# manips-sai-org/sai-primitives

Measured on AMD Instinct MI355X. Metric: control-cycles/sec (whole node), 7-DoF 2-task hierarchy, batch=4096, higher is better.
Workload: dtype f64

## Files before the change

### sai-primitives_amd/csrc/saip_kernel_oct.hip

```cpp
#include <hip/hip_runtime.h>
#include <math.h>

#include "saip_device.h"
#include "saip_dynamics_oct_body.h"
#include "saip_fk.h"
#include "saip_law.h"
#include "saip_oct_common.h"
#define SAIP_WG_SYNC()                                          \
	do {                                                        \
		__builtin_amdgcn_fence(__ATOMIC_RELEASE, "wavefront");  \
		__builtin_amdgcn_wave_barrier();                        \
		__builtin_amdgcn_fence(__ATOMIC_ACQUIRE, "wavefront");  \
	} while (0)
#include "saip_wg_cycle.h"

namespace saip {

#if defined(SAIP_STAMP_OCT)
__device__ unsigned long long saip_stamps_oct[1024 * 64];
#define STAMP(i)                                                                              \
	do {                                                                                      \
		__builtin_amdgcn_sched_barrier(0);                                                    \
		if (blockIdx.x < 1024 && (threadIdx.x & 63) == 0) saip_stamps_oct[blockIdx.x * 64 + (threadIdx.x >> 6) * 32 + (i)] = __builtin_amdgcn_s_memtime(); \
		__builtin_amdgcn_sched_barrier(0);                                                    \
	} while (0)
#else
#define STAMP(i)
#endif

struct OctInst {
	union {
		double X[8][12];
		struct {
			double T1[6][8], A[8][8], Am[8][8], Lam[8][8];
			double N1[8][8];
		};
	};
	double M[8][8];
	double zo[8][6];
	double J[6][8];
	double vec[13][8];
	double ist[10];
};
static_assert(sizeof(OctInst) % 256 == 16, "instance stride must be 2 (mod 32) doubles");
static_assert(sizeof(OctInst) * 8 * 4 <= 160 * 1024, "four wavefronts per CU (one LDS block each, also with two wavefronts per instance group)");

template <int R>
__device__ __forceinline__ void oct_jacobi_n(double (&A)[R][R], double (&V)[R][R], const int lane) {
	static_assert(R == 4 || R == 6, "even sizes with at most three pairs per round");
	constexpr int NP = R / 2, RM = R - 1;
	const int r = octl_r(lane), m = r & 1;
	auto rotation = [](const double apq, const double app, const double aqq, double& cs, double& sn, double& tn) {
		const double d = aqq - app, b2 = 2.0 * apq;
		const double x = fma(d, d, b2 * b2);
		const bool rot = x > 1e-300;
		const double h = rot ? x * oct_rsqrt(x) : 1.0;
		const double tm = fabs(b2) * oct_rcp(fabs(d) + h);
		tn = rot ? (((d >= 0.0) == (b2 >= 0.0)) ? tm : -tm) : 0.0;
		cs = oct_rsqrt(fma(tn, tn, 1.0));
		sn = tn * cs;
	};
	double vrow[R];
	UNR for (int j = 0; j < R; j++) vrow[j] = (j == r) ? 1.0 : 0.0;
	for (int sweep = 0; sweep < 12; sweep++) {
		double off = 0.0, dg = 0.0;
		UNR for (int p = 0; p < R; p++) {
			dg = fma(A[p][p], A[p][p], dg);
			UNR for (int q = p + 1; q < R; q++) off = fma(A[p][q], A[p][q], off);
		}
		if (!__any(off > 1e-32 * dg)) break;
		UNR for (int t = 0; t < RM; t++) {
			double apq = 0.0, app = 0.0, aqq = 0.0;
			UNR for (int j = 0; j < NP; j++) {
				const int a_ = j == 0 ? t : (t + j) % RM, b_ = j == 0 ? RM : (t + RM - j) % RM;
				const int p = a_ < b_ ? a_ : b_, q = a_ < b_ ? b_ : a_;
				const bool mine = m == j;
				apq = mine ? A[p][q] : apq;
				app = mine ? A[p][p] : app;
				aqq = mine ? A[q][q] : aqq;
			}
			double cs, sn, tn, cs2 = 1.0, sn2 = 0.0, tn2 = 0.0;
			rotation(apq, app, aqq, cs, sn, tn);
			if (NP == 3) {
				const int a_ = (t + 2) % RM, b_ = (t + RM - 2) % RM;
				const int p = a_ < b_ ? a_ : b_, q = a_ < b_ ? b_ : a_;
				rotation(A[p][q], A[p][p], A[q][q], cs2, sn2, tn2);
			}
			UNR for (int j = 0; j < NP; j++) {
				const int a_ = j == 0 ? t : (t + j) % RM, b_ = j == 0 ? RM : (t + RM - j) % RM;
				const int p = a_ < b_ ? a_ : b_, q = a_ < b_ ? b_ : a_;
				double c, s_, tj;
				if (j == 0) { c = oct_dpp<0x44>(cs); s_ = oct_dpp<0x44>(sn); tj = oct_dpp<0x44>(tn); }
				else if (j == 1) { c = oct_dpp<0xEE>(cs); s_ = oct_dpp<0xEE>(sn); tj = oct_dpp<0xEE>(tn); }
				else { c = cs2; s_ = sn2; tj = tn2; }
				const double apq_j = A[p][q];
				UNR for (int k = 0; k < R; k++) {
					if (k != p && k != q) {
						const double akp = A[k][p], akq = A[k][q];
						const double np_ = c * akp - s_ * akq, nq_ = s_ * akp + c * akq;
						A[k][p] = np_;
						A[p][k] = np_;
						A[k][q] = nq_;
						A[q][k] = nq_;
					}
				}
				A[p][p] = fma(-tj, apq_j, A[p][p]);
				A[q][q] = fma(tj, apq_j, A[q][q]);
				A[p][q] = 0.0;
				A[q][p] = 0.0;
				const double vp = vrow[p], vq = vrow[q];
				vrow[p] = c * vp - s_ * vq;
				vrow[q] = s_ * vp + c * vq;
			}
		}
	}
	UNR for (int i = 0; i < R; i++)
		UNR for (int c = 0; c < R; c++) V[i][c] = __shfl(vrow[c], octl_src(lane, i));
}
__device__ __forceinline__ void oct_jacobi4(double (&A)[4][4], double (&V)[4][4], const int lane) { oct_jacobi_n<4>(A, V, lane); }
__device__ __forceinline__ void oct_spd_inverse4(const double (&A)[4][4], double (&Ainv)[4][4]) { oct_spd_inverse_n<4>(A, Ainv); }


__device__ __forceinline__ void oct_fk_frame(const ModelDev& md, const int rr, const int r, const double q, double (&Tw)[12]) {
	const double* R0 = md.R0[rr];
	const double ax = md.axis[rr][0], ay = md.axis[rr][1], az = md.axis[rr][2];
	if (md.jtype[rr] == 1) {
		double s, c;
		sincos_joint(q, &s, &c);
		const double v = 1.0 - c;
		const double Rq[9] = {c + ax * ax * v,      ax * ay * v - az * s, ax * az * v + ay * s,
							  ay * ax * v + az * s, c + ay * ay * v,      ay * az * v - ax * s,
							  az * ax * v - ay * s, az * ay * v + ax * s, c + az * az * v};
		UNR for (int i = 0; i < 3; i++)
			UNR for (int j = 0; j < 3; j++) Tw[3 * i + j] = R0[3 * i] * Rq[j] + R0[3 * i + 1] * Rq[3 + j] + R0[3 * i + 2] * Rq[6 + j];
		UNR for (int e = 0; e < 3; e++) Tw[9 + e] = md.p0[rr][e];
	} else {
		UNR for (int e = 0; e < 9; e++) Tw[e] = R0[e];
		const double a[3] = {ax, ay, az};
		double d[3];
		oct_mat3_vec(R0, a, d);
		UNR for (int e = 0; e < 3; e++) Tw[9 + e] = md.p0[rr][e] + d[e] * q;
	}
	OCT_FRAME_STEP(1, Tw)
	OCT_FRAME_STEP(2, Tw)
	OCT_FRAME_STEP(4, Tw)
}


template <bool DUO>
__device__ __forceinline__ void oct_sync() {
	if (DUO) {
		__builtin_amdgcn_fence(__ATOMIC_RELEASE, "wavefront");
		__builtin_amdgcn_wave_barrier();
		__builtin_amdgcn_fence(__ATOMIC_ACQUIRE, "wavefront");
	} else {
		__syncthreads();
	}
}

template <bool FULL, int GJ, int ROLE, int NN = 7>
__device__ __forceinline__ bool oct_cycle_body(const CycleParams& P, OctInst* smem, OctInst* smemA, OctInst* smemB, int* wgflags = nullptr, double* lawc = nullptr) {
	constexpr bool DUO = ROLE != 0;
	constexpr bool roleA = ROLE != 2, roleB = ROLE != 1;
	constexpr int N = NN;
	constexpr bool CF = !FULL && GJ == 0;
	constexpr bool BROWS = DUO && CF;
	auto flag_wait = [&](const int k) {
		int it = 0, v = 0;
		while ((v = __hip_atomic_load(wgflags + k, __ATOMIC_RELAXED, __HIP_MEMORY_SCOPE_WORKGROUP)) == 0 && ++it < 200000) __builtin_amdgcn_s_sleep(1);
		__builtin_amdgcn_fence(__ATOMIC_ACQUIRE, "workgroup");
		return v;
	};
	auto flag_set = [&](const int k, const int v) {
		__builtin_amdgcn_fence(__ATOMIC_RELEASE, "workgroup");
		if ((threadIdx.x & 63) == 0) __hip_atomic_store(wgflags + k, v, __ATOMIC_RELAXED, __HIP_MEMORY_SCOPE_WORKGROUP);
	};
	bool lost = false;
	static_assert(NN == 7 || (FULL && GJ == 2), "6- and 8-dof chains: the general instantiation only");
	const int lane = threadIdx.x & 63;
	const int r = octl_r(lane), grp = octl_grp(lane);
	const int rr = r < N ? r : N - 1;
	const bool act = r < N;
	OctInst& sm = smem[grp];
	OctInst& smA = smemA[grp];
	OctInst& smB = smemB[grp];
	const int b_raw = (int)blockIdx.x * 8 + grp;
	const bool live = b_raw < P.B;
	const int b = live ? b_raw : P.B - 1;
	const size_t ld = P.ld;
	const ModelDev& md = *P.model;
	const TaskDev& mf = P.tasks[0];
	const TaskDev& jt = P.tasks[1];
	const int kmf = FULL ? mf.k : 6;
	const int mf_dec_v = mf.decoupling, jt_dec_v = jt.decoupling;
	const bool trunc_mode = FULL && GJ == 2 && P.oct_truncate;

	STAMP(0);
	const double q_r = P.q[(size_t)rr * ld + b];
	const double dq_r = P.dq[(size_t)rr * ld + b];
	const int jtype_r = md.jtype[rr];
	double R0v[9], p0v[3], axv[3];
	UNR for (int e = 0; e < 9; e++) R0v[e] = md.R0[rr][e];
	UNR for (int e = 0; e < 3; e++) {
		p0v[e] = md.p0[rr][e];
		axv[e] = md.axis[rr][e];
	}
	double comv[3] = {0, 0, 0}, inev[6] = {0, 0, 0, 0, 0, 0}, mass_r = 0.0;
	if (ROLE == 0) {
		UNR for (int e = 0; e < 3; e++) comv[e] = md.com[rr][e];
		UNR for (int e = 0; e < 6; e++) inev[e] = md.inertia[rr][e];
		mass_r = md.mass[rr];
	}
	double gl0 = 0.0, gl1 = 0.0, gl2 = 0.0;
	if (roleB) {
		gl0 = saip_ldg(P.goal2[0], (size_t)r * ld + b);
		gl1 = saip_ldg(P.goal2[0], (size_t)(8 + r) * ld + b);
		gl2 = saip_ldg(P.goal2[0], (size_t)(16 + r) * ld + b);
	}
	const double gl3 = (roleB && FULL && mf.general_law && r < 6) ? saip_ldg(P.goal2[0], (size_t)(24 + r) * ld + b) : 0.0;
	static_assert(offsetof(TaskDev, Ppos) == offsetof(TaskDev, Bm) + 36 * 8 && offsetof(TaskDev, Pori) == offsetof(TaskDev, Bm) + 45 * 8 &&
					  offsetof(TaskDev, sig_p) == offsetof(TaskDev, Bm) + 54 * 8 && offsetof(TaskDev, sig_o) == offsetof(TaskDev, Bm) + 63 * 8 &&
					  offsetof(TaskDev, kp_pos) == offsetof(TaskDev, Bm) + 72 * 8 && offsetof(TaskDev, ki_ori) == offsetof(TaskDev, Bm) + 87 * 8,
				  "the law constants are one contiguous run");
	double lc0 = 0.0, lc1 = 0.0;
	if (FULL && roleB) {
		const double* lsrc = reinterpret_cast<const double*>(reinterpret_cast<const char*>(&mf) + offsetof(TaskDev, Bm));
		lc0 = lsrc[lane];
		lc1 = lsrc[lane < 26 ? 64 + lane : 89];
	}
	const int mj = GJ == 1 ? jt.m : N;
	const int rj = GJ == 1 ? (r < mj ? r : 0) : rr;
	double jg_q = 0.0, jg_dq = 0.0, jg_ddq = 0.0;
	if (roleA) {
		jg_q = saip_ldg(P.goal2[1], (size_t)rj * ld + b);
		jg_dq = saip_ldg(P.goal2[1], (size_t)(mj + rj) * ld + b);
		jg_ddq = saip_ldg(P.goal2[1], (size_t)(2 * mj + rj) * ld + b);
	}

#define OCT_REQUEST_STATE(SFX)                                                                                          \
	const bool track_mf##SFX = (mf.has_ki || P.integ_always), track_jt##SFX = (jt.has_ki || P.integ_always);            \
	double mfi_pre##SFX = 0.0, jti_pre##SFX = 0.0;                                                                      \
	if (roleB && track_mf##SFX && r < 6) mfi_pre##SFX = saip_ldg(P.integ2[0], (size_t)r * ld + b);                                   \
	if (roleA && track_jt##SFX) jti_pre##SFX = saip_ldg(P.integ2[1], (size_t)(GJ == 1 ? rj : rr) * ld + b);                          \
	double jkp_r##SFX = 0.0, jkv_r##SFX = 0.0, jki_r##SFX = 0.0;  \
	if (roleA && GJ != 1) {                                                                                             \
		jkp_r##SFX = jt.kp[rr];                                                                                         \
		jkv_r##SFX = jt.kv[rr];                                                                                         \
		jki_r##SFX = jt.ki[rr];                                                                                         \
	}
	double jt_ie_new = 0.0;
	OCT_REQUEST_STATE(_e)

	STAMP(1);
	double Tw[12];
	{
		const double* R0 = R0v;
		const double ax = axv[0], ay = axv[1], az = axv[2];
		if (jtype_r == 1) {
			double s, c;
			sincos_joint(q_r, &s, &c);
			if (md.all_axis_z) {
				UNR for (int i = 0; i < 3; i++) {
					Tw[3 * i] = R0[3 * i] * c + R0[3 * i + 1] * s;
					Tw[3 * i + 1] = R0[3 * i + 1] * c - R0[3 * i] * s;
					Tw[3 * i + 2] = R0[3 * i + 2];
				}
			} else {
				const double v = 1.0 - c;
				const double Rq[9] = {c + ax * ax * v,      ax * ay * v - az * s, ax * az * v + ay * s,
									  ay * ax * v + az * s, c + ay * ay * v,      ay * az * v - ax * s,
									  az * ax * v - ay * s, az * ay * v + ax * s, c + az * az * v};
				UNR for (int i = 0; i < 3; i++)
					UNR for (int j = 0; j < 3; j++) Tw[3 * i + j] = R0[3 * i] * Rq[j] + R0[3 * i + 1] * Rq[3 + j] + R0[3 * i + 2] * Rq[6 + j];
			}
			UNR for (int e = 0; e < 3; e++) Tw[9 + e] = p0v[e];
		} else {
			UNR for (int e = 0; e < 9; e++) Tw[e] = R0[e];
			const double a[3] = {ax, ay, az};
			double d[3];
// ... 100 lines not shown
		const double c0 = z[1] * rz - z[2] * ry, c1 = z[2] * rx - z[0] * rz, c2 = z[0] * ry - z[1] * rx;
		const double jw[6] = {on ? (rev ? c0 : z[0]) : 0.0, on ? (rev ? c1 : z[1]) : 0.0, on ? (rev ? c2 : z[2]) : 0.0,
							  (on && rev) ? z[0] : 0.0,    (on && rev) ? z[1] : 0.0,    (on && rev) ? z[2] : 0.0};
		UNR for (int a = 0; a < 6; a++) jwc[a] = act ? jw[a] : 0.0;
		if (FULL && !mf.bm_identity) {
			UNR for (int a = 0; a < 6; a++) {
				double sj = 0.0;
				UNR for (int e = 0; e < 6; e++) sj = fma(lawc[e * 6 + a], jw[e], sj);
				sm.J[a][r] = sj;
			}
		} else {
			UNR for (int a = 0; a < 6; a++) sm.J[a][r] = jw[a];
		}
	}
	double fi_pre = 0.0;
	if (roleA && GJ != 1) {
		const double e = q_r - jg_q;
		double ie = track_jt ? jti_pre : 0.0;
		ie += e * jt.dt;
		jt_ie_new = ie;
		if (jt.vel_sat) {
			double vdes = -jkp_r * jt.kvinv[rr] * e - jki_r * jt.kvinv[rr] * ie;
			vdes = fmin(fmax(vdes, -jt.sat[rr]), jt.sat[rr]);
			fi_pre = -jkv_r * (dq_r - vdes);
		} else {
			fi_pre = -jkp_r * e - jkv_r * (dq_r - jg_dq) - jki_r * ie;
		}
	}
	if (BROWS) oct_sync<DUO>();
	else if (DUO && !trunc_mode) __syncthreads();
	else oct_sync<DUO>();
	STAMP(3);
	double mi[N] = {}, mb[N] = {};
	int eclamp = 0;
	double cclamp = 0.0;
	bool general_bie = false;
	if (roleA) {
		double L[N][N], dinv[N];
		UNR for (int i = 0; i < N; i++)
			UNR for (int j = 0; j <= i; j++) L[i][j] = sm.M[i][j];
		if (P.any_bie) {
			int nclamp = 0;
			UNR for (int e = 0; e < N; e++) {
				const double ce = P.bie_thr - L[e][e];
				if (ce > 0.0) {
					nclamp++;
					eclamp = e;
					cclamp = ce;
				}
			}
			general_bie = __any(nclamp > 1);
		}
		if (general_bie) {
			double Lb[N][N], dinvb[N];
			UNR for (int i = 0; i < N; i++)
				UNR for (int j = 0; j <= i; j++) Lb[i][j] = (i == j) ? fmax(L[i][j], P.bie_thr) : L[i][j];
			oct_cholesky<N>(L, dinv);
			oct_cholesky<N>(Lb, dinvb);
			oct_solve_unit<N>(L, dinv, rr, mi);
			oct_solve_unit<N>(Lb, dinvb, rr, mb);
		} else {
			oct_cholesky<N>(L, dinv);
			oct_solve_unit<N>(L, dinv, rr, mi);
			UNR for (int j = 0; j < N; j++) mb[j] = mi[j];
		}
	}
	const bool rank1_bie = P.any_bie && !general_bie;
	auto park_minv = [&]() {
		if (ROLE == 1) {
			UNR for (int j = 0; j < N; j++) sm.N1[r][j] = mi[j];
		}
		if (roleA && rank1_bie && r == eclamp) {
			UNR for (int j = 0; j < N; j++) sm.vec[3][j] = mi[j];
		}
	};
	if (!CF) park_minv();
	STAMP(4);
	double Jf[6][N];
	unsigned keep_bits_b = 0x3fu;
	if (DUO && trunc_mode && ROLE == 1) {
		__syncthreads();
		keep_bits_b = (unsigned)smB.vec[6][7];
	}
	if (!(BROWS && ROLE == 1)) {
		UNR for (int a = 0; a < 6; a++)
			UNR for (int j = 0; j < N; j++) Jf[a][j] = (ROLE == 1 ? smB : sm).J[a][j];
	}
	double vw[6] = {0, 0, 0, 0, 0, 0};
	if (roleB) {
		double dqa[N];
		UNR for (int j = 0; j < N; j++) dqa[j] = sm.vec[0][j];
		UNR for (int a = 0; a < 6; a++) {
			double s = 0.0;
			UNR for (int j = 0; j < N; j++) s = fma(Jf[a][j], dqa[j], s);
			vw[a] = s;
		}
		if (FULL && !mf.bm_identity) {
			UNR for (int a = 0; a < 6; a++) vw[a] = octl_sum(jwc[a] * dq_r);
		}
	}
	STAMP(5);
	double Fum6[6], Ff6[6] = {0, 0, 0, 0, 0, 0};
	STAMP(6);
	bool singular = false, truncated = false, blended_i = false;
	const bool strategies_on = GJ == 0 && mf.sing_handling && mf.sing_strategies && mf.sh != nullptr;
	double G[6][6], U6[6][6];
	bool keepm[6] = {true, true, true, true, true, true};
	double LG[6][6], dG[6];
	double zcf[N] = {}, wcf[N] = {}, zzcf = 0.0;
	auto form_z = [&](const double (&Lg)[6][6], const double (&dg)[6]) {
		double jc6[6], x6[6], xb[6], prr = 1.0;
		UNR for (int a = 0; a < 6; a++) jc6[a] = (ROLE == 1 ? smB : sm).J[a][rr];
		oct_solve<6>(Lg, dg, jc6, x6);
		UNR for (int a = 0; a < 6; a++) prr = fma(-jc6[a], x6[a], prr);
		double bestw = act ? prr : -1.0;
		int jbw = r;
#define OCT_ARGMAX_STEP(CTRL)                                                                                   \
	{                                                                                                           \
		const double ob = oct_dpp<CTRL>(bestw);                                                                 \
		const int oj = __builtin_amdgcn_update_dpp(0, jbw, CTRL, 0xF, 0xF, true);                               \
		const bool take = ob > bestw || (ob == bestw && oj < jbw);                                              \
		bestw = take ? ob : bestw;                                                                              \
		jbw = take ? oj : jbw;                                                                                  \
	}
		OCT_ARGMAX_STEP(OCT_BFLY0)
		OCT_ARGMAX_STEP(OCT_BFLY1)
		OCT_ARGMAX_STEP(OCT_BFLY2)
#undef OCT_ARGMAX_STEP
		const int src = octl_src(lane, jbw);
		UNR for (int a = 0; a < 6; a++) xb[a] = __shfl(x6[a], src);
		double z_own = (rr == jbw) ? 1.0 : 0.0;
		UNR for (int a = 0; a < 6; a++) z_own = fma(-jc6[a], xb[a], z_own);
		UNR for (int j = 0; j < N; j++) {
			zcf[j] = __shfl(z_own, octl_src(lane, j));
			zzcf = fma(zcf[j], zcf[j], zzcf);
		}
	};
	auto run_law = [&]() {
		double ip[3] = {0, 0, 0}, io[3] = {0, 0, 0}, Fum[6], G24[24];
		UNR for (int e = 0; e < 24; e++) G24[e] = sm.vec[10 + (e >> 3)][e & 7];
		if (track_mf) {
			UNR for (int i = 0; i < 3; i++) {
				ip[i] = sm.ist[i];
				io[i] = sm.ist[3 + i];
			}
		}
		if (FULL && mf.general_law) {
			double G30[30], Ff[6] = {0, 0, 0, 0, 0, 0};
			UNR for (int e = 0; e < 24; e++) G30[e] = G24[e];
			UNR for (int e = 0; e < 6; e++) G30[24 + e] = sm.vec[5][e];
			law_motion_force_general<false>(&mf, vw, pw, Rc, G30, ip, io, (double*)nullptr, Fum, Ff);
			UNR for (int a = 0; a < 6; a++) Ff6[a] = Ff[a];
		} else if (FULL && !mf.bm_identity) {
			double v[3], w[3], e3[3], tmp[3], Fw[6];
			UNR for (int i = 0; i < 3; i++) {
				v[i] = lawc[36 + 3 * i] * vw[0] + lawc[36 + 3 * i + 1] * vw[1] + lawc[36 + 3 * i + 2] * vw[2];
				w[i] = lawc[45 + 3 * i] * vw[3] + lawc[45 + 3 * i + 1] * vw[4] + lawc[45 + 3 * i + 2] * vw[5];
			}
			UNR for (int i = 0; i < 3; i++) e3[i] = pw[i] - G24[i];
			UNR for (int i = 0; i < 3; i++) ip[i] += (lawc[54 + 3 * i] * e3[0] + lawc[54 + 3 * i + 1] * e3[1] + lawc[54 + 3 * i + 2] * e3[2]) * mf.dt;
			UNR for (int i = 0; i < 3; i++) tmp[i] = G24[18 + i] - lawc[72 + i] * e3[i] - lawc[75 + i] * (v[i] - G24[12 + i]) - lawc[78 + i] * ip[i];
			UNR for (int i = 0; i < 3; i++) Fw[i] = lawc[54 + 3 * i] * tmp[0] + lawc[54 + 3 * i + 1] * tmp[1] + lawc[54 + 3 * i + 2] * tmp[2];
			double oe[3] = {0, 0, 0};
			UNR for (int c = 0; c < 3; c++) {
				const double a0 = Rc[c], a1 = Rc[3 + c], a2 = Rc[6 + c], b0 = G24[3 + c], b1 = G24[6 + c], b2 = G24[9 + c];
				oe[0] -= 0.5 * (a1 * b2 - a2 * b1);
				oe[1] -= 0.5 * (a2 * b0 - a0 * b2);
				oe[2] -= 0.5 * (a0 * b1 - a1 * b0);
			}
			double dphi[3];
			UNR for (int i = 0; i < 3; i++) dphi[i] = lawc[63 + 3 * i] * oe[0] + lawc[63 + 3 * i + 1] * oe[1] + lawc[63 + 3 * i + 2] * oe[2];
			UNR for (int i = 0; i < 3; i++) io[i] += dphi[i] * mf.dt;
			UNR for (int i = 0; i < 3; i++) tmp[i] = G24[21 + i] - lawc[81 + i] * dphi[i] - lawc[84 + i] * (w[i] - G24[15 + i]) - lawc[87 + i] * io[i];
			UNR for (int i = 0; i < 3; i++) Fw[3 + i] = lawc[63 + 3 * i] * tmp[0] + lawc[63 + 3 * i + 1] * tmp[1] + lawc[63 + 3 * i + 2] * tmp[2];
			UNR for (int a = 0; a < 6; a++) {
				double sf = 0.0;
				UNR for (int e = 0; e < 6; e++) sf = fma(lawc[0 + e * 6 + a], Fw[e], sf);
				Fum[a] = sf;
			}
		} else {
		double e3[3];
		UNR for (int i = 0; i < 3; i++) e3[i] = pw[i] - G24[i];
		UNR for (int i = 0; i < 3; i++) ip[i] = fma(e3[i], mf.dt, ip[i]);
		UNR for (int i = 0; i < 3; i++) Fum[i] = G24[18 + i] - mf.kp_pos[i] * e3[i] - mf.kv_pos[i] * (vw[i] - G24[12 + i]) - mf.ki_pos[i] * ip[i];
		double oe[3] = {0, 0, 0};
		UNR for (int c = 0; c < 3; c++) {
			const double a0 = Rc[c], a1 = Rc[3 + c], a2 = Rc[6 + c], b0 = G24[3 + c], b1 = G24[6 + c], b2 = G24[9 + c];
			oe[0] -= 0.5 * (a1 * b2 - a2 * b1);
			oe[1] -= 0.5 * (a2 * b0 - a0 * b2);
			oe[2] -= 0.5 * (a0 * b1 - a1 * b0);
		}
		UNR for (int i = 0; i < 3; i++) io[i] = fma(oe[i], mf.dt, io[i]);
		UNR for (int i = 0; i < 3; i++) Fum[3 + i] = G24[21 + i] - mf.kp_ori[i] * oe[i] - mf.kv_ori[i] * (vw[3 + i] - G24[15 + i]) - mf.ki_ori[i] * io[i];
		}
		if (track_mf && r == 0) {
			UNR for (int i = 0; i < 3; i++) {
				sm.ist[i] = ip[i];
				sm.ist[3 + i] = io[i];
			}
		}
		if (trunc_mode) {
			double fh[6];
			UNR for (int a = 0; a < 6; a++) {
				double sf = 0.0;
				UNR for (int i = 0; i < 6; i++) sf = fma(U6[i][a], Fum[i], sf);
				fh[a] = keepm[a] ? sf : 0.0;
			}
			UNR for (int a = 0; a < 6; a++) Fum[a] = fh[a];
		}
		UNR for (int a = 0; a < 6; a++) Fum6[a] = Fum[a];
	};
	if (roleB && CF) run_law();
	if (roleB) {
		double tr = 0.0;
		UNR for (int a = 0; a < 6; a++)
			UNR for (int c = 0; c <= a; c++) {
				double s = 0.0;
				UNR for (int j = 0; j < N; j++) s = fma(Jf[a][j], Jf[c][j], s);
				G[a][c] = s;
				G[c][a] = s;
				if (a == c) tr += s;
			}
		if (CF) {
			UNR for (int a = 0; a < 6; a++)
				UNR for (int c = 0; c <= a; c++) LG[a][c] = G[a][c];
			oct_cholesky<6>(LG, dG);
			if (ROLE == 2) {
				if (r == 0) {
					UNR for (int a = 0; a < 6; a++) {
						UNR for (int c = 0; c <= a; c++) sm.Lam[a][c] = LG[a][c];
						sm.Lam[6][a] = dG[a];
					}
				}
				flag_set(0, 1);
			}
			double y6[6];
			if (mf_dec == DEC_IMPEDANCE) {
				UNR for (int a = 0; a < 6; a++) y6[a] = Fum6[a];
			} else {
				oct_solve<6>(LG, dG, Fum6, y6);
			}
			UNR for (int j = 0; j < N; j++) {
				double s = 0.0;
				UNR for (int a = 0; a < 6; a++) s = fma(Jf[a][j], y6[a], s);
				wcf[j] = s;
			}
			if (ROLE == 0) form_z(LG, dG);
			UNR for (int j = 0; j < N; j++) {
				if (ROLE == 0) asm volatile("" : "+v"(zcf[j]));
				asm volatile("" : "+v"(wcf[j]));
			}
			if (ROLE == 0) asm volatile("" : "+v"(zzcf));
		}
		const double itr = oct_rcp(tr);
		const double smax2 = mf.s_max * mf.s_max, tol2 = mf.s_abs_tol * mf.s_abs_tol;
		auto ldl_positive = [&](const double shift) {
			double Gs[6][6];
			UNR for (int a = 0; a < 6; a++)
				UNR for (int c = 0; c <= a; c++) Gs[a][c] = G[a][c] * itr;
			bool pos = true;
			UNR for (int a = 0; a < 6; a++) Gs[a][a] = (a < kmf) ? Gs[a][a] - shift : 1.0;
			UNR for (int kk = 0; kk < 6; kk++) {
				const double d = Gs[kk][kk];
				pos = pos && (d > 1e-13);
				const double id = oct_rcp(d);
				UNR for (int i = kk + 1; i < 6; i++) {
					const double lik = Gs[i][kk] * id;
					UNR for (int j = kk + 1; j <= i; j++) Gs[i][j] = fma(-lik, Gs[j][kk], Gs[i][j]);
				}
			}
			return pos;
		};
		bool need_exact = !((tr > 0.0) && (tr >= (double)kmf * tol2) && ldl_positive(smax2));
#if defined(SAIP_OCT_FORCE_EXACT)
		need_exact = true;
#endif
		if (__any(need_exact)) {
			double G2[6][6], Gt[6][6];
			UNR for (int a = 0; a < 6; a++)
				UNR for (int c = 0; c < 6; c++) G2[a][c] = G[a][c] * itr;
			UNR for (int rep = 0; rep < 2; rep++) {
				UNR for (int a = 0; a < 6; a++)
					UNR for (int c = 0; c <= a; c++) {
						double s = 0.0;
						UNR for (int l = 0; l < 6; l++) s = fma(G2[a][l], G2[l][c], s);
						Gt[a][c] = s;
					}
				UNR for (int a = 0; a < 6; a++)
					UNR for (int c = 0; c <= a; c++) {
						G2[a][c] = Gt[a][c];
						G2[c][a] = Gt[a][c];
					}
			}
			double t8 = 0.0;
			UNR for (int a = 0; a < 6; a++)
				UNR for (int c = 0; c < 6; c++) t8 = fma(G2[a][c], G2[a][c], t8);
			const double u = sqrt(sqrt(sqrt(t8)));
			const bool ok_s0 = (u * mf.cert_kroot * tr >= tol2);
			const bool pos = ldl_positive(smax2 * u);
			need_exact = need_exact && !(ok_s0 && pos && tr > 0.0);
			if (need_exact) {
				double lmx = 0.0;
				UNR for (int a = 0; a < 6; a++) lmx = (a < kmf) ? fmax(lmx, G[a][a] * itr) : lmx;
				double Gs[6][6];
				UNR for (int a = 0; a < 6; a++)
					UNR for (int c = 0; c <= a; c++) Gs[a][c] = G[a][c] * itr;
				UNR for (int a = 0; a < 6; a++) Gs[a][a] = (a < kmf) ? Gs[a][a] - smax2 * lmx : 1.0;
				bool neg = false, clean = true;
				UNR for (int kk = 0; kk < 6; kk++) {
					const double dpv = Gs[kk][kk];
					neg = neg || (clean && dpv < -1e-12);
					clean = clean && (dpv > 1e-13);
					const double id = oct_rcp(dpv);
					UNR for (int i = kk + 1; i < 6; i++) {
						const double lik = Gs[i][kk] * id;
						UNR for (int j = kk + 1; j <= i; j++) Gs[i][j] = fma(-lik, Gs[j][kk], Gs[i][j]);
					}
				}
				if ((tr > 0.0 && neg) || tr < tol2) {
					singular = true;
					need_exact = false;
				}
			}
#if defined(SAIP_OCT_FORCE_EXACT)
			need_exact = true;
#endif
			if (strategies_on && need_exact) {
				singular = true;
				need_exact = false;
			}
			if (__any(need_exact)) {
				if (need_exact && r == 0) {
					for (int a = 0; a < 6; a++)
						for (int c = 0; c < 6; c++) sm.A[a][c] = G[a][c];
					oct_serial_jacobi(&sm.A[0][0], nullptr, kmf, 8);
// ... 148 lines not shown
			UNR for (int a = 0; a < 6; a++) {
				double sacc = 0.0;
				UNR for (int l = 0; l < N; l++) sacc = fma(Jf[a][l], mcol[l], sacc);
				t[a] = sacc;
				lt_own = fma(lam[a], sacc, lt_own);
			}
			sm.vec[4][r] = lt_own;
			oct_sync<DUO>();
			double lt[6], q = 0.0;
			UNR for (int a = 0; a < 6; a++) {
				lt[a] = sm.vec[4][a];
				q = fma(t[a], lt[a], q);
			}
			const double gamma = beta * oct_rcp(fma(-beta, q, 1.0));
			UNR for (int c = 0; c < 6; c++) lmod[c] = fma(gamma * lt_own, lt[c], lam[c]);
		}
	}
	if (GJ != 0) {
		UNR for (int c = 0; c < 6; c++) sm.Lam[r][c] = lam[c];
	}
	STAMP(9);
	if (roleB && !CF) run_law();
	if (DUO && !CF) {
		if (ROLE == 2) {
			if (r < 6) {
				double fo = 0.0, ffo = 0.0;
				UNR for (int a = 0; a < 6; a++) {
					fo = (a == r) ? Fum6[a] : fo;
					ffo = (a == r) ? Ff6[a] : ffo;
				}
				sm.vec[6][r] = fo;
				sm.vec[5][r] = ffo;
			}
			if (r == 6) sm.vec[6][6] = (singular ? 1.0 : 0.0) + (truncated ? 2.0 : 0.0);
		}
		STAMP(29);
		__syncthreads();
		STAMP(30);
		if (ROLE == 2 && GJ != 0) return false;
		if (ROLE == 1) {
			UNR for (int a = 0; a < 6; a++) {
				Fum6[a] = smB.vec[6][a];
				Ff6[a] = smB.vec[5][a];
			}
			if (GJ != 0) {
				const int fl = (int)smB.vec[6][6];
				singular = (fl & 1) != 0;
				truncated = (fl & 2) != 0;
			}
		}
		if (GJ == 0) {
			UNR for (int i = 0; i < 6; i++)
				UNR for (int j = 0; j <= i; j++) L6[i][j] = smA.A[i][j];
			oct_cholesky<6>(L6, dinv6);
			if (ROLE == 2) {
				UNR for (int a = 0; a < 6; a++) t1c[a] = smA.T1[a][r];
				UNR for (int j = 0; j < N; j++) mi[j] = smA.N1[r][j];
			}
		}
	}
	if (GJ != 0) {
		double s = 0.0;
		UNR for (int a = 0; a < 6; a++) s = (a == ra) ? Ff6[a] : s;
		UNR for (int c = 0; c < 6; c++) s = fma(lmod[c], Fum6[c], s);
		sm.vec[2][r] = s;
		oct_sync<DUO>();
	}
	STAMP(10);
	double tau_r;
	double cj[N];
	double cn = 0.0;
	double tv;
	if (GJ == 0) {
		double g[6];
		double wr = 0.0;
		tau_r = 0.0;
		double v[N] = {}, zr = 0.0, v_own = 0.0, zz = 0.0, zv = 0.0;
		double fi = 0.0;
		double tvo = 0.0;
		bool ovr = false;
		int hand = 1;
		if (CF) {
			double wv[N] = {};
			if (roleB) {
				UNR for (int j = 0; j < N; j++) wv[j] = wcf[j];
			}
			if (ROLE == 2) {
				hand = (strategies_on && __any(singular)) ? 2 : 1;
				if (r == 0) {
					UNR for (int j = 0; j < N; j++) sm.vec[8][j] = wv[j];
				}
				sm.vec[2][r] = singular ? 2.0 : 0.0;
				STAMP(29);
				flag_set(1, hand);
			}
			if (ROLE == 1) {
				double Lg[6][6], dg[6];
				if (flag_wait(0) == 0) lost = true;
				STAMP(12);
				UNR for (int a = 0; a < 6; a++) {
					UNR for (int c = 0; c <= a; c++) Lg[a][c] = smB.Lam[a][c];
					dg[a] = smB.Lam[6][a];
				}
				form_z(Lg, dg);
			}
			double mrow[N], pr = 0.0, sr = 0.0, z_r = 0.0, mrr = 0.0, mi_rr = 0.0, c_r = 0.0, cm = 0.0, mxz = 0.0, s2 = 1.0, mu = 1.0, rho = 1.0;
			if (roleA) {
				UNR for (int j = 0; j < N; j++) v[j] = zcf[j];
				zz = zzcf;
				UNR for (int j = 0; j < N; j++) mrow[j] = (j <= rr) ? sm.M[rr][j] : sm.M[j][rr];
				UNR for (int j = 0; j < N; j++) {
					pr = fma(mrow[j], v[j], pr);
					sr = fma(mi[j], v[j], sr);
					z_r = (j == rr) ? v[j] : z_r;
					mrr = (j == rr) ? mrow[j] : mrr;
					mi_rr = (j == rr) ? mi[j] : mi_rr;
				}
				c_r = P.any_bie ? fmax(P.bie_thr - mrr, 0.0) : 0.0;
				cm = (mf_dec == DEC_BIE) ? c_r : 0.0;
				mxz = fma(cm, z_r, pr);
				const double zl = act ? z_r : 0.0;
				s2 = octl_sum(zl * mxz);
				mu = octl_sum(zl * pr);
				if (jt_dec == DEC_IMPEDANCE) {
					rho = zz * oct_rcp(mu);
				} else if (jt_dec == DEC_BIE) {
					if (general_bie) {
						double zcz = 0.0, mbcz = 0.0;
						UNR for (int j = 0; j < N; j++) {
							const double czj = fmax(P.bie_thr - sm.M[j][j], 0.0) * v[j];
							zcz = fma(czj, v[j], zcz);
							mbcz = fma(mb[j], czj, mbcz);
						}
						const double qb = octl_sum(act ? c_r * z_r * mbcz : 0.0);
						rho = mu * oct_rcp(mu - zcz + qb);
					} else {
						const double mee = __shfl(mi_rr, octl_src(lane, eclamp));
						const double bcf = cclamp * oct_rcp(fma(cclamp, mee, 1.0));
						double ze = 0.0;
						UNR for (int j = 0; j < N; j++) ze = (j == eclamp) ? v[j] : ze;
						rho = mu * oct_rcp(fma(-bcf * ze, ze, mu));
					}
				}
			}
			if (ROLE == 1) {
				STAMP(13);
				hand = __builtin_amdgcn_readfirstlane(flag_wait(1));
				STAMP(30);
				lost = lost || hand == 0;
				UNR for (int j = 0; j < N; j++) wv[j] = smB.vec[8][j];
				singular = ((int)smB.vec[2][r] & 2) != 0;
				if (__builtin_expect(hand == 2, 0)) {
					UNR for (int a = 0; a < 6; a++)
						UNR for (int j = 0; j < N; j++) Jf[a][j] = smB.J[a][j];
					park_minv();
					form_t1_a();
					flag_set(2, 1);
				}
			}
			if (roleA) {
				double mw = 0.0, w_r = 0.0;
				UNR for (int j = 0; j < N; j++) {
					mw = fma(mrow[j], wv[j], mw);
					w_r = (j == rr) ? wv[j] : w_r;
				}
				const double mxw = fma(cm, w_r, mw);
				const double s1 = octl_sum(act ? z_r * mxw : 0.0);
				tau_r = (mf_dec == DEC_IMPEDANCE) ? w_r : fma(-mxz, s1 * oct_rcp(s2), mxw);
				fi = fi_pre;
				const double sj = octl_sum(act ? fma(rho * z_r, fi, fma(z_r, jg_ddq, -sr * tau_r)) : 0.0);
				tv = fma(pr * oct_rcp(zz), sj, tau_r);
			}
		} else {
		if (roleA) {
// ... 17 lines not shown
					t[a] = sacc;
				}
				oct_solve<6>(L6, dinv6, t, y2);
				UNR for (int a = 0; a < 6; a++) {
					ty1 = fma(t[a], y1[a], ty1);
					ty2 = fma(t[a], y2[a], ty2);
				}
				const double gamma = beta * oct_rcp(fma(-beta, ty2, 1.0));
				UNR for (int a = 0; a < 6; a++) g[a] = fma(gamma * ty1, y2[a], y1[a]) + Ff6[a];
			} else {
				UNR for (int a = 0; a < 6; a++) g[a] = y1[a] + Ff6[a];
			}
		}
		double tau1[N];
		UNR for (int j = 0; j < N; j++) {
			double s = 0.0;
			UNR for (int a = 0; a < 6; a++) s = fma(Jf[a][j], g[a], s);
			tau1[j] = s;
			wr = fma(mi[j], s, wr);
		}
		UNR for (int j = 0; j < N; j++) tau_r = (j == rr) ? tau1[j] : tau_r;
		}
		if (roleB) {
		double x6[6], rowv[N], nr = 0.0;
		oct_solve<6>(L6, dinv6, t1c, x6);
		UNR for (int j = 0; j < N; j++) {
			double acc = (j == rr) ? 1.0 : 0.0;
			UNR for (int a = 0; a < 6; a++) acc = fma(-Jf[a][j], x6[a], acc);
			rowv[j] = acc;
			nr = fma(acc, acc, nr);
		}
		double bestw = act ? nr : -1.0;
		int jbw = r;
#define OCT_ARGMAX_STEP(CTRL)                                                                                   \
	{                                                                                                           \
		const double ob = oct_dpp<CTRL>(bestw);                                                                 \
		const int oj = __builtin_amdgcn_update_dpp(0, jbw, CTRL, 0xF, 0xF, true);                               \
		const bool take = ob > bestw || (ob == bestw && oj < jbw);                                              \
		bestw = take ? ob : bestw;                                                                              \
		jbw = take ? oj : jbw;                                                                                  \
	}
		OCT_ARGMAX_STEP(OCT_BFLY0)
		OCT_ARGMAX_STEP(OCT_BFLY1)
		OCT_ARGMAX_STEP(OCT_BFLY2)
#undef OCT_ARGMAX_STEP
		const int src = octl_src(lane, jbw);
		UNR for (int j = 0; j < N; j++) {
			v[j] = __shfl(rowv[j], src);
			zr = fma(mi[j], v[j], zr);
			v_own = (j == rr) ? v[j] : v_own;
		}
		zr = act ? zr : 0.0;
		zz = octl_sum(zr * zr);
		zv = octl_sum(zr * v_own);
		}
		if (roleA) {
		fi = fi_pre;
		}
		if (ROLE == 0) {
		const double ai = jg_ddq - wr;
		const double za = octl_sum(zr * ai);
		const double zf = octl_sum(zr * fi);
		double rho = 1.0;
		if (jt_dec == DEC_IMPEDANCE) {
			rho = zz * oct_rcp(zv);
		} else if (jt_dec == DEC_BIE) {
			if (general_bie) {
				if (DUO) {
					UNR for (int j = 0; j < N; j++) v[j] = smB.vec[4][j];
				}
				double mbv = 0.0;
				UNR for (int j = 0; j < N; j++) mbv = fma(mb[j], v[j], mbv);
				const double qb = octl_sum(act ? v_own * mbv : 0.0);
				rho = zv * oct_rcp(qb);
			} else {
				const double ze = octl_sum((act && r == eclamp) ? zr : 0.0);
				rho = zv * oct_rcp(fma(-beta * ze, ze, zv));
			}
		}
		tv = fma(v_own * oct_rcp(zz), fma(rho, zf, za), tau_r);
		}
		}
		if (ROLE != 1 && __builtin_expect(strategies_on && __any(singular), 0)) {
			if (CF && ROLE == 0) {
				park_minv();
				form_t1_a();
			}
			if (ROLE == 2) {
				if (CF) {
					if (flag_wait(2) == 0) lost = true;
					UNR for (int j = 0; j < N; j++) mi[j] = smA.N1[r][j];
				}
				eclamp = (int)smA.vec[9][1];
				general_bie = smA.vec[9][2] != 0.0;
				beta = smA.vec[9][0];
				const bool r1b = P.any_bie && !general_bie;
				UNR for (int j = 0; j < N; j++) mcol[j] = r1b ? smA.vec[3][j] : 0.0;
				UNR for (int j = 0; j < N; j++) mb[j] = general_bie ? smA.Lam[r][j] : mi[j];
				jg_q = saip_ldg(P.goal2[1], (size_t)rr * ld + b);
				jg_dq = saip_ldg(P.goal2[1], (size_t)(N + rr) * ld + b);
				jg_ddq = saip_ldg(P.goal2[1], (size_t)(2 * N + rr) * ld + b);
				const double e = q_r - jg_q;
				double ie = 0.0;
				if (jt.has_ki || P.integ_always) ie = saip_ldg(P.integ2[1], (size_t)rr * ld + b);
				ie += e * jt.dt;
				if (jt.vel_sat) {
					double vdes = -jt.kp[rr] * jt.kvinv[rr] * e - jt.ki[rr] * jt.kvinv[rr] * ie;
					vdes = fmin(fmax(vdes, -jt.sat[rr]), jt.sat[rr]);
					fi = -jt.kv[rr] * (dq_r - vdes);
				} else {
					fi = -jt.kp[rr] * e - jt.kv[rr] * (dq_r - jg_dq) - jt.ki[rr] * ie;
				}
			}
			STAMP(16);
			double Ue[6][6], sig[6], ju[6];
			bool keep[6];
			double smax = 0.0;
			double trg = 0.0;
			{
				double E[6][6];
				UNR for (int a = 0; a < 6; a++)
					UNR for (int c = 0; c <= a; c++) {
						double sacc = 0.0;
						UNR for (int j = 0; j < N; j++) sacc = fma(Jf[a][j], Jf[c][j], sacc);
						E[a][c] = sacc;
						E[c][a] = sacc;
						if (a == c) trg += sacc;
					}
				oct_jacobi_n<6>(E, Ue, lane);
			}
			STAMP(17);
			double tu[6];
			UNR for (int c = 0; c < 6; c++) {
				double s2 = 0.0, own = 0.0, tacc = 0.0;
				UNR for (int j = 0; j < N; j++) {
					double acc = 0.0;
					UNR for (int i = 0; i < 6; i++) acc = fma(Ue[i][c], Jf[i][j], acc);
					s2 = fma(acc, acc, s2);
					own = (j == rr) ? acc : own;
					tacc = fma(acc, mcol[j], tacc);
				}
				tu[c] = tacc;
				sig[c] = sqrt(s2);
				smax = fmax(smax, sig[c]);
				ju[c] = own;
			}
			STAMP(18);
			int ns = 0, cstar = 0;
			double sstar = -1.0;
			bool tiny = false;
			UNR for (int c = 0; c < 6; c++) {
				keep[c] = sig[c] >= mf.s_max * smax;
				ns += keep[c] ? 1 : 0;
				if (!keep[c] && sig[c] > sstar) {
					sstar = sig[c];
					cstar = c;
				}
				tiny = tiny || (!keep[c] && !(sig[c] >= 1e-10 * smax));
			}
			const bool finite_state = (trg - trg == 0.0);
			const bool fully = finite_state && !(smax >= mf.s_abs_tol);
			const bool blend = singular && finite_state && !fully && ns < 6 && !tiny;
			const bool clear = singular && finite_state && !fully && ns == 6;
			if (clear) singular = false;
			if (__any(singular && fully)) {
				double acc = 0.0;
// ... 693 lines not shown
		const double ai = jg_ddq - wr;
		double a1[5], b1[5];
		UNR for (int c = 0; c < 5; c++) {
			a1[c] = octl_sum(uown[c] * ai);
			b1[c] = octl_sum(uown[c] * fi);
		}
		double tj = tau_r;
		UNR for (int c = 0; c < 5; c++) {
			double gc = 0.0;
			UNR for (int k5 = 0; k5 < 5; k5++) gc = fma(Lam5[c][k5], a1[k5], fma(Lmod5[c][k5], b1[k5], gc));
			tj = fma(jh[c], (c < rank) ? gc : 0.0, tj);
		}
		tv = tj;
	}
	}
	STAMP(14);
	if (P.torque_sat) {
		const double lim = md.effort[rr];
		tv = tv > lim ? lim : (tv < -lim ? -lim : tv);
	}
	if (FULL && P.jla) {
		bool zone;
		const double tj = jla_joint(q_r, dq_r, md.q_lower[rr], md.q_upper[rr], md.vel_limit[rr], md.effort[rr], tv, &zone);
		const bool in_zone = zone && act && !singular;
		if (__any(in_zone)) {
			sm.vec[1][r] = tv;
			sm.vec[3][r] = in_zone ? 1.0 : 0.0;
			oct_sync<DUO>();
			double tall[N], zall[N];
			UNR for (int j = 0; j < N; j++) {
				tall[j] = sm.vec[1][j];
				zall[j] = sm.vec[3][j];
			}
			double sacc = 0.0;
			UNR for (int j = 0; j < N; j++) sacc = fma(mi[j], tall[j], sacc);
			sm.vec[4][r] = in_zone ? sacc : 0.0;
			UNR for (int j = 0; j < N; j++) sm.N1[r][j] = (in_zone && zall[j] != 0.0) ? mi[j] : ((j == rr) ? 1.0 : 0.0);
			oct_sync<DUO>();
			double L[N][N], dinv[N], y[N], x[N];
			UNR for (int i = 0; i < N; i++)
				UNR for (int j = 0; j <= i; j++) L[i][j] = sm.N1[i][j];
			oct_cholesky<N>(L, dinv);
			UNR for (int i = 0; i < N; i++) {
				double sy = sm.vec[4][i];
				UNR for (int k = 0; k < i; k++) sy = fma(-L[i][k], y[k], sy);
				y[i] = sy * dinv[i];
			}
			UNR for (int i = N - 1; i >= 0; i--) {
				double sx = y[i];
				UNR for (int k = i + 1; k < N; k++) sx = fma(-L[k][i], x[k], sx);
				x[i] = sx * dinv[i];
			}
			double yr = 0.0;
			UNR for (int i = 0; i < N; i++) yr = (i == rr) ? x[i] : yr;
			if (in_zone) tv = tj + tv - yr;
			if (P.torque_sat) {
				const double lim = md.effort[rr];
				tv = tv > lim ? lim : (tv < -lim ? -lim : tv);
			}
		}
	}
	if (P.gravity_comp) {
		const double* gv = md.gravity;
		const double ax_ = Ic[1] - Ic[0] * o[0], ay_ = Ic[2] - Ic[0] * o[1], az_ = Ic[3] - Ic[0] * o[2];
		const double cx = z[1] * az_ - z[2] * ay_, cy = z[2] * ax_ - z[0] * az_, cz = z[0] * ay_ - z[1] * ax_;
		const double tgr = -(cx * gv[0] + cy * gv[1] + cz * gv[2]);
		const double tgp = -Ic[0] * (z[0] * gv[0] + z[1] * gv[1] + z[2] * gv[2]);
		tv += rev ? tgr : tgp;
	}
	const bool to_tail = GJ != 0 && P.slow_tail && singular;
	if (live && act && !singular) P.tau[(size_t)r * ld + b] = tv;
	if (live && act && singular && P.flag_nan && !to_tail) P.tau[(size_t)r * ld + b] = __builtin_nan("");
	if (live && r == 0 && !to_tail) P.status[b] = singular ? 1 : ((truncated ? 2 : 0) | (blended_i ? 8 : 0));
	if (live && r == 0 && singular && P.flag_list) {
		const int slot = atomicAdd(P.flag_count, 1);
		if (slot < P.B) P.flag_list[slot] = b;
	}
	if (P.flag_list && blockIdx.x == 0 && lane == 0) *P.flag_count_next = 0;
	if (live && !singular) {
		if (track_mf && r < 6) P.integ2[0][(size_t)r * ld + b] = (ROLE == 1 ? smB : sm).ist[r];
		if (track_jt && (GJ == 1 ? r < mj : act)) P.integ2[1][(size_t)r * ld + b] = jt_ie_new;
	}
	STAMP(15);
	return live && to_tail;
}

__device__ __forceinline__ void oct_slow_tail(const CycleParams& P, const bool flagged, void* lds) {
	const unsigned long long votes = __ballot(flagged);
	if (__builtin_expect(votes == 0ull, 1)) return;
	static_assert(sizeof(WgSmem<8>) <= 8 * sizeof(OctInst), "the general kernel's block fits the eight instance blocks of a wavefront");
	WgSmem<8>& wsm = *reinterpret_cast<WgSmem<8>*>(lds);
	for (int g = 0; g < 8; g++) {
		const int l0 = ((g >> 1) << 4) | (g & 1);
		if (((votes >> l0) & 1ull) == 0ull) continue;
		SAIP_WG_SYNC();
		wg_cycle<8, 64>(P, (int)blockIdx.x * 8 + g, wsm);
	}
}

template <bool FULL, int GJ, bool DUO = false, bool SIM = false, int NN = 7>
__global__ void __launch_bounds__(DUO ? 128 : 64) saip_cycle_oct(const CycleParams P) {
	static_assert(!SIM || NN == 7, "the fused integration step is the 7-dof one");
	__shared__ OctInst smem[DUO ? 16 : 8];
	static_assert(sizeof(OctInst) >= sizeof(OctDynInst), "the integration step reuses the cycle's LDS blocks");
	const bool wave_b = DUO && __builtin_amdgcn_readfirstlane((int)(threadIdx.x >> 6)) == 1;
	__shared__ int wgflags[3];
	__shared__ double lawc[FULL ? 96 : 1];
	if (DUO && !FULL && GJ == 0) {
		if (threadIdx.x == 0) wgflags[0] = wgflags[1] = wgflags[2] = 0;
		__syncthreads();
	}
	bool flagged = false;
	if (DUO) {
		if (wave_b) oct_cycle_body<FULL, GJ, DUO ? 2 : 0, NN>(P, smem + 8, smem, smem + 8, wgflags, lawc);
		else flagged = oct_cycle_body<FULL, GJ, DUO ? 1 : 0, NN>(P, smem, smem, smem + 8, wgflags, lawc);
	} else {
		flagged = oct_cycle_body<FULL, GJ, 0, NN>(P, smem, smem, smem, nullptr, lawc);
	}
	if (GJ != 0 && !SIM && !wave_b) oct_slow_tail(P, flagged, smem);
	if (SIM && !wave_b) {
		SimParams S;
		S.B = P.B;
		S.ld = P.ld;
		S.n = P.n;
		S.substeps = P.sim_substeps;
		S.dt = P.sim_dt;
		S.damping = P.sim_damping;
		S.gravity[0] = P.sim_gravity[0];
		S.gravity[1] = P.sim_gravity[1];
		S.gravity[2] = P.sim_gravity[2];
		S.model = P.model;
		S.q = const_cast<double*>(P.q);
		S.dq = const_cast<double*>(P.dq);
		S.tau = P.tau;
		S.ddq = nullptr;
		integrate_oct_body(S, reinterpret_cast<OctDynInst*>(DUO ? smem + 8 : smem), (int)blockIdx.x, (int)(threadIdx.x & 63));
	}
}

static bool oct_duo_enabled(const int workgroups) {
	static int cus = 0;
	if (cus == 0) {
		int dev = 0, n = 0;
		if (hipGetDevice(&dev) != hipSuccess || hipDeviceGetAttribute(&n, hipDeviceAttributeMultiprocessorCount, dev) != hipSuccess || n <= 0) n = 256;
		cus = n;
	}
	return workgroups <= 2 * cus;
}

hipError_t launch_cycle_oct(const CycleParams& P, hipStream_t stream) {
	const dim3 grid((P.B + 7) / 8), block(64);
	const bool duo = oct_duo_enabled((int)grid.x);
	if (P.oct_general_joint == 2 && P.n == 8) {
		if (duo) hipLaunchKernelGGL((saip_cycle_oct<true, 2, true, false, 8>), grid, dim3(128), 0, stream, P);
		else hipLaunchKernelGGL((saip_cycle_oct<true, 2, false, false, 8>), grid, block, 0, stream, P);
	} else if (P.oct_general_joint == 2 && P.n == 6) {
		if (duo) hipLaunchKernelGGL((saip_cycle_oct<true, 2, true, false, 6>), grid, dim3(128), 0, stream, P);
		else hipLaunchKernelGGL((saip_cycle_oct<true, 2, false, false, 6>), grid, block, 0, stream, P);
	} else if (P.oct_general_joint == 2) {
		if (duo) hipLaunchKernelGGL((saip_cycle_oct<true, 2, true>), grid, dim3(128), 0, stream, P);
		else hipLaunchKernelGGL((saip_cycle_oct<true, 2>), grid, block, 0, stream, P);
	} else if (P.oct_general_joint == 1) {
		if (duo) hipLaunchKernelGGL((saip_cycle_oct<true, 1, true>), grid, dim3(128), 0, stream, P);
		else hipLaunchKernelGGL((saip_cycle_oct<true, 1>), grid, block, 0, stream, P);
	} else if (P.jla || P.lane_general || P.oct_partial_mf) {
		if (P.sim_substeps > 0) {
// ... 21 lines not shown
```

Measured before the change: 510.9 million.

## Distribute J Gram matrix and task-velocity dot products across lanes via LDS

In the closed-form path, each lane now computes only three entries of the 6x6 Gram matrix J·Jᵀ and one component of J·dq, using a fixed pair table checked at compile time. The partial results are exchanged through shared memory after a sync, so lanes no longer each compute the full 21-entry Gram and hold the whole 6xN Jacobian in registers. The dynamically consistent w vector is likewise reduced to one element per lane and then gathered from LDS. This trades redundant per-lane FMAs and register pressure for extra LDS traffic and synchronisation, and the full Jacobian is reloaded only on the rare singular path. Realtime timestamp probes are also added but are compiled only under the stamp build flag.

```diff
diff --git a/sai-primitives_amd/csrc/saip_kernel_oct.hip b/sai-primitives_amd/csrc/saip_kernel_oct.hip
--- a/sai-primitives_amd/csrc/saip_kernel_oct.hip
+++ b/sai-primitives_amd/csrc/saip_kernel_oct.hip
@@ -24,8 +24,13 @@
 		if (blockIdx.x < 1024 && (threadIdx.x & 63) == 0) saip_stamps_oct[blockIdx.x * 64 + (threadIdx.x >> 6) * 32 + (i)] = __builtin_amdgcn_s_memtime(); \
 		__builtin_amdgcn_sched_barrier(0);                                                    \
 	} while (0)
+#define STAMP_RT(i)                                                                                                                   \
+	do {                                                                                                                              \
+		if (blockIdx.x < 1024 && threadIdx.x == 0) saip_stamps_oct[blockIdx.x * 64 + 32 + (i)] = __builtin_amdgcn_s_memrealtime();   \
+	} while (0)
 #else
 #define STAMP(i)
+#define STAMP_RT(i)
 #endif
 
 struct OctInst {
@@ -44,6 +49,25 @@
 };
 static_assert(sizeof(OctInst) % 256 == 16, "instance stride must be 2 (mod 32) doubles");
 static_assert(sizeof(OctInst) * 8 * 4 <= 160 * 1024, "four wavefronts per CU (one LDS block each, also with two wavefronts per instance group)");
+
+constexpr unsigned OCT_G_P1 = 0x43254321u, OCT_G_P2 = 0x55005432u;
+__host__ __device__ constexpr int oct_g_own(const int l) { return l < 6 ? l : l - 6; }
+__host__ __device__ constexpr int oct_g_word(const int a, const int c) {
+	if (a == c) return a;
+	for (int l = 0; l < 8; l++) {
+		const int o = oct_g_own(l), p1 = (int)((OCT_G_P1 >> (4 * l)) & 7u), p2 = (int)((OCT_G_P2 >> (4 * l)) & 7u);
+		if ((o == a && p1 == c) || (o == c && p1 == a)) return 8 + l;
+		if ((o == a && p2 == c) || (o == c && p2 == a)) return 16 + l;
+	}
+	return -1;
+}
+__host__ __device__ constexpr bool oct_g_map_complete() {
+	for (int a = 0; a < 6; a++)
+		for (int c = 0; c < a; c++)
+			if (oct_g_word(a, c) < 0) return false;
+	return true;
+}
+static_assert(oct_g_map_complete(), "every pair of rows of J has a lane");
 
 template <int R>
 __device__ __forceinline__ void oct_jacobi_n(double (&A)[R][R], double (&V)[R][R], const int lane) {
@@ -195,6 +219,7 @@
 	const int mf_dec_v = mf.decoupling, jt_dec_v = jt.decoupling;
 	const bool trunc_mode = FULL && GJ == 2 && P.oct_truncate;
 
+	if (ROLE != 2) STAMP_RT(12);
 	STAMP(0);
 	const double q_r = P.q[(size_t)rr * ld + b];
 	const double dq_r = P.dq[(size_t)rr * ld + b];
@@ -461,12 +486,46 @@
 		__syncthreads();
 		keep_bits_b = (unsigned)smB.vec[6][7];
 	}
-	if (!(BROWS && ROLE == 1)) {
+	if (!CF) {
 		UNR for (int a = 0; a < 6; a++)
 			UNR for (int j = 0; j < N; j++) Jf[a][j] = (ROLE == 1 ? smB : sm).J[a][j];
 	}
 	double vw[6] = {0, 0, 0, 0, 0, 0};
-	if (roleB) {
+	double G[6][6];
+	double jcol[6] = {0, 0, 0, 0, 0, 0};
+	if (roleB && CF) {
+		const int own = oct_g_own(r), p1 = (int)((OCT_G_P1 >> (4 * r)) & 7u), p2 = (int)((OCT_G_P2 >> (4 * r)) & 7u);
+		double jo[N], j1[N], j2[N], dqa[N];
+		UNR for (int j = 0; j < N; j++) {
+			jo[j] = sm.J[own][j];
+			j1[j] = sm.J[p1][j];
+			j2[j] = sm.J[p2][j];
+			dqa[j] = sm.vec[0][j];
+		}
+		UNR for (int a = 0; a < 6; a++) jcol[a] = sm.J[a][rr];
+		double g0 = 0.0, g1 = 0.0, g2 = 0.0, v0 = 0.0;
+		UNR for (int j = 0; j < N; j++) {
+			v0 = fma(jo[j], dqa[j], v0);
+			g0 = fma(jo[j], jo[j], g0);
+			g1 = fma(jo[j], j1[j], g1);
+			g2 = fma(jo[j], j2[j], g2);
+		}
+		sm.Am[0][r] = g0;
+		sm.Am[1][r] = g1;
+		sm.Am[2][r] = g2;
+		sm.Am[3][r] = v0;
+		oct_sync<DUO>();
+		UNR for (int a = 0; a < 6; a++) {
+			vw[a] = sm.Am[3][a];
+			UNR for (int c = 0; c <= a; c++) {
+				const int e = oct_g_word(a, c);
+				const double s = sm.Am[e >> 3][e & 7];
+				G[a][c] = s;
+				G[c][a] = s;
+			}
+		}
+	}
+	if (roleB && !CF) {
 		double dqa[N];
 		UNR for (int j = 0; j < N; j++) dqa[j] = sm.vec[0][j];
 		UNR for (int a = 0; a < 6; a++) {
@@ -483,10 +542,11 @@
 	STAMP(6);
 	bool singular = false, truncated = false, blended_i = false;
 	const bool strategies_on = GJ == 0 && mf.sing_handling && mf.sing_strategies && mf.sh != nullptr;
-	double G[6][6], U6[6][6];
+	double U6[6][6];
 	bool keepm[6] = {true, true, true, true, true, true};
 	double LG[6][6], dG[6];
-	double zcf[N] = {}, wcf[N] = {}, zzcf = 0.0;
+	double zcf[N] = {}, zzcf = 0.0;
+	double w_own = 0.0;
 	auto form_z = [&](const double (&Lg)[6][6], const double (&dg)[6]) {
 		double jc6[6], x6[6], xb[6], prr = 1.0;
 		UNR for (int a = 0; a < 6; a++) jc6[a] = (ROLE == 1 ? smB : sm).J[a][rr];
@@ -592,14 +652,18 @@
 	if (roleB && CF) run_law();
 	if (roleB) {
 		double tr = 0.0;
-		UNR for (int a = 0; a < 6; a++)
-			UNR for (int c = 0; c <= a; c++) {
-				double s = 0.0;
-				UNR for (int j = 0; j < N; j++) s = fma(Jf[a][j], Jf[c][j], s);
-				G[a][c] = s;
-				G[c][a] = s;
-				if (a == c) tr += s;
-			}
+		if (CF) {
+			UNR for (int a = 0; a < 6; a++) tr += G[a][a];
+		} else {
+			UNR for (int a = 0; a < 6; a++)
+				UNR for (int c = 0; c <= a; c++) {
+					double s = 0.0;
+					UNR for (int j = 0; j < N; j++) s = fma(Jf[a][j], Jf[c][j], s);
+					G[a][c] = s;
+					G[c][a] = s;
+					if (a == c) tr += s;
+				}
+		}
 		if (CF) {
 			UNR for (int a = 0; a < 6; a++)
 				UNR for (int c = 0; c <= a; c++) LG[a][c] = G[a][c];
@@ -619,17 +683,14 @@
 			} else {
 				oct_solve<6>(LG, dG, Fum6, y6);
 			}
-			UNR for (int j = 0; j < N; j++) {
-				double s = 0.0;
-				UNR for (int a = 0; a < 6; a++) s = fma(Jf[a][j], y6[a], s);
-				wcf[j] = s;
-			}
+			UNR for (int a = 0; a < 6; a++) w_own = fma(jcol[a], y6[a], w_own);
 			if (ROLE == 0) form_z(LG, dG);
 			UNR for (int j = 0; j < N; j++) {
 				if (ROLE == 0) asm volatile("" : "+v"(zcf[j]));
-				asm volatile("" : "+v"(wcf[j]));
-			}
+			}
+			asm volatile("" : "+v"(w_own));
 			if (ROLE == 0) asm volatile("" : "+v"(zzcf));
+			sm.vec[8][r] = w_own;
 		}
 		const double itr = oct_rcp(tr);
 		const double smax2 = mf.s_max * mf.s_max, tol2 = mf.s_abs_tol * mf.s_abs_tol;
@@ -944,14 +1005,12 @@
 		int hand = 1;
 		if (CF) {
 			double wv[N] = {};
-			if (roleB) {
-				UNR for (int j = 0; j < N; j++) wv[j] = wcf[j];
+			if (ROLE == 0) {
+				oct_sync<DUO>();
+				UNR for (int j = 0; j < N; j++) wv[j] = sm.vec[8][j];
 			}
 			if (ROLE == 2) {
 				hand = (strategies_on && __any(singular)) ? 2 : 1;
-				if (r == 0) {
-					UNR for (int j = 0; j < N; j++) sm.vec[8][j] = wv[j];
-				}
 				sm.vec[2][r] = singular ? 2.0 : 0.0;
 				STAMP(29);
 				flag_set(1, hand);
@@ -1135,6 +1194,10 @@
 		}
 		}
 		if (ROLE != 1 && __builtin_expect(strategies_on && __any(singular), 0)) {
+			if (CF) {
+				UNR for (int a = 0; a < 6; a++)
+					UNR for (int j = 0; j < N; j++) Jf[a][j] = sm.J[a][j];
+			}
 			if (CF && ROLE == 0) {
 				park_minv();
 				form_t1_a();
@@ -1994,6 +2057,7 @@
 		if (track_jt && (GJ == 1 ? r < mj : act)) P.integ2[1][(size_t)r * ld + b] = jt_ie_new;
 	}
 	STAMP(15);
+	if (ROLE != 2) STAMP_RT(13);
 	return live && to_tail;
 }
 
```

Result: faster. 521.6 million (median of 6 runs) (+2.1%).
